# sailab-code/GNN_tf_2.x

Hardware: AMD Instinct MI355X
Metric: node-state-updates/sec (nodes x iters / s), 1M-node synthetic graph (higher is better)
Workload: dtype f32; 1 GPU; synthetic randomGraph-recipe graph, N=1000000 nodes, E=9999690 arcs, state_dim=64, net_state 135->128->128->64 selu+BN, net_output 67->2 softmax+BN, max_iter=30, threshold=0 (all iterations run); the loop-invariant label aggregates (GNN.py:259, :263; 0.2 ms) are kept between Loops until the labels change, see cold_aggregates_ms_per_step; parallelism=single GPU, tile_form=one wave per 32-node tile (k_fused)

## Files before the change

### gnn_tf_2.x_amd/csrc/gnn_fused_kernel.h

```cpp
#pragma once
#include <utility>

#include "gnn_common.h"
#include "gnn_fused.h"

typedef float f32x16 __attribute__((ext_vector_type(16)));

namespace gnn_fused_dev {

#define GNN_GLOBAL __attribute__((address_space(1)))
template <class T>
__device__ __forceinline__ const GNN_GLOBAL T *gptr(const T *p) { return (const GNN_GLOBAL T *)p; }
template <class T>
__device__ __forceinline__ GNN_GLOBAL T *gptr_w(T *p) { return (GNN_GLOBAL T *)p; }
typedef float v4f __attribute__((ext_vector_type(4)));
typedef float v2f __attribute__((ext_vector_type(2)));
typedef int v4i_ __attribute__((ext_vector_type(4)));
__device__ __forceinline__ v4f gload4(const float *p) { return *(const GNN_GLOBAL v4f *)p; }
#ifndef GNN_STORE_AUX
#define GNN_STORE_AUX 2
#endif
__device__ __forceinline__ void gstore_row4(float *base, int64_t off, v4f v)
{
#if GNN_STORE_AUX == 0
// ... 223 lines not shown
#undef GNN_L0_LOAD
#undef GNN_L0_MFMA
}

template <int ACT>
struct ActPipe2 {
    v2f t, u, n, f, p, e;
    static __device__ __forceinline__ v2f splat(float c) { return v2f{c, c}; }
    __device__ __forceinline__ void stage(int st, float v0, float v1, float b0, float b1, float &o0, float &o1)
    {
        if constexpr (ACT == GNN_ACT_SELU) {
            switch (st) {
            case 0: t = v2f{v0, v1} + v2f{b0, b1}; u = t * splat(1.44269504088896341f); break;
            case 1: n = v2f{__builtin_rintf(u.x), __builtin_rintf(u.y)}; f = u - n; break;
            case 2: p = __builtin_elementwise_fma(splat(0.0013218672247603536f), f, splat(0.009671698324382305f));
                    p = __builtin_elementwise_fma(p, f, splat(0.05550893023610115f)); break;
            case 3: p = __builtin_elementwise_fma(p, f, splat(0.24022237956523895f));
                    p = __builtin_elementwise_fma(p, f, splat(0.6931468844413757f)); break;
            case 4: p = __builtin_elementwise_fma(p, f, splat(1.0f)); break;
            case 5: e = v2f{__builtin_ldexpf(p.x, (int)n.x), __builtin_ldexpf(p.y, (int)n.y)}; e = e - splat(1.0f); break;
            case 6: e = e * splat(1.6732632423543772f); break;
            case 7: {
                const v2f r = v2f{t.x > 0.0f ? t.x : e.x, t.y > 0.0f ? t.y : e.y} * splat(1.0507009873554805f);
                o0 = r.x; o1 = r.y;
            } break;
            }
        } else {
            if (st == 0) t = v2f{v0, v1} + v2f{b0, b1};
            if (st == 7) { o0 = gnn_act(t.x, ACT); o1 = gnn_act(t.y, ACT); }
        }
    }
};

template <int NI, int NO, int ACT>
__device__ __forceinline__ void layer_from_regs(f32x16 (&hin)[NI], const float *bias_prev, int half, f32x16 (&acc)[NO],
                                                const float *wp, int wstride)
{
    constexpr int STEPS = 16 * NI, DEPTH = 8;
    float w[STEPS][NO];
#pragma unroll
    for (int s = 0; s < DEPTH; ++s) load_w<NO>(wp + (size_t)s * 64 * NO * wstride, w[s]);
    tile_epilogue<ACT, false>(hin[0], bias_prev, nullptr, nullptr, 0, half);
    acc_to_operand(hin[0]);
    __builtin_amdgcn_sched_barrier(0);
#pragma unroll
    for (int ti = 0; ti < NI; ++ti) {
        float nb[16];
        if (ti + 1 < NI) {
#pragma unroll
            for (int q = 0; q < 4; ++q) {
                const v4f b4 = gload4(bias_prev + 32 * (ti + 1) + 8 * q + 4 * half);
                nb[4 * q] = b4.x; nb[4 * q + 1] = b4.y; nb[4 * q + 2] = b4.z; nb[4 * q + 3] = b4.w;
            }
        }
        __builtin_amdgcn_sched_barrier(0);
        ActPipe2<ACT> ap;
#pragma unroll
        for (int ss = 0; ss < 16; ++ss) {
            const int s = 16 * ti + ss;
            if (s + DEPTH < STEPS) load_w<NO>(wp + (size_t)(s + DEPTH) * 64 * NO * wstride, w[s + DEPTH]);
            const int reg = 4 * (ss >> 2) + ((ss & 3) == 1 ? 2 : (ss & 3) == 2 ? 1 : (ss & 3));
            const float b = hin[ti][reg];
            const bool epi = ti + 1 < NI;
            const int pe = ss & ~1;
#pragma unroll
            for (int jt = 0; jt < NO; ++jt) {
                acc[jt] = __builtin_amdgcn_mfma_f32_32x32x2f32(w[s][jt], b, acc[jt], 0, 0, 0);
                if (epi) {
                    constexpr int SPM = 4 / NO;
#pragma unroll
                    for (int q = jt * SPM; q < (jt + 1) * SPM; ++q) {
                        const int st = (ss & 1) * 4 + q;
                        float o0 = 0.0f, o1 = 0.0f;
                        ap.stage(st, hin[ti + 1][pe], hin[ti + 1][pe + 1], nb[pe], nb[pe + 1], o0, o1);
                        if (st == 7) {
                            auto sw = __builtin_amdgcn_permlane32_swap(__float_as_uint(o0), __float_as_uint(o1), false, false);
                            hin[ti + 1][pe] = __uint_as_float(sw[0]);
                            hin[ti + 1][pe + 1] = __uint_as_float(sw[1]);
                        }
                    }
                }
                __builtin_amdgcn_sched_barrier(0);
            }
            __builtin_amdgcn_sched_barrier(0);
        }
    }
}

typedef int v4i __attribute__((ext_vector_type(4)));
typedef __bf16 bf16x8 __attribute__((ext_vector_type(8)));
__device__ __forceinline__ v4i gload4i(const int *p) { return *(const GNN_GLOBAL v4i *)p; }

__device__ __forceinline__ v4i bload4i(__amdgpu_buffer_rsrc_t r, int voff, int soff)
{
    return __builtin_bit_cast(v4i, __builtin_amdgcn_raw_buffer_load_b128(r, voff, soff, 0));
}
struct WStream {
    int soff, n;
    __device__ __forceinline__ WStream(int start) : soff(start), n(0) {}
    __device__ __forceinline__ v4i next(__amdgpu_buffer_rsrc_t r, int voff)
    {
        if (n == 4) { asm volatile("s_add_u32 %0, %0, 0x1000" : "+s"(soff) : : "scc"); n = 0; }
        return bload4i(r, voff + 1024 * n++, soff);
    }
};

__device__ __forceinline__ f32x16 bias_tile(const float *bias_lds, int jt, int half)
{
    f32x16 t;
#pragma unroll
    for (int q = 0; q < 4; ++q) {
        const v4f b = *reinterpret_cast<const v4f *>(bias_lds + 32 * jt + 8 * q + 4 * half);
        t[4 * q] = b.x; t[4 * q + 1] = b.y; t[4 * q + 2] = b.z; t[4 * q + 3] = b.w;
    }
    return t;
}

__device__ __forceinline__ void split8(const float (&v)[8], v4i &p0, v4i &p1, v4i &p2)
{
#pragma unroll
    for (int j = 0; j < 4; ++j) {
        const unsigned a = __float_as_uint(v[2 * j]), b = __float_as_uint(v[2 * j + 1]);
        const float ar = v[2 * j] - __uint_as_float(a & 0xffff0000u), br = v[2 * j + 1] - __uint_as_float(b & 0xffff0000u);
        const unsigned aru = __float_as_uint(ar), bru = __float_as_uint(br);
        const float ar2 = ar - __uint_as_float(aru & 0xffff0000u), br2 = br - __uint_as_float(bru & 0xffff0000u);
        p0[j] = (int)__builtin_amdgcn_perm(b, a, 0x07060302u);
        p1[j] = (int)__builtin_amdgcn_perm(bru, aru, 0x07060302u);
        p2[j] = (int)__builtin_amdgcn_perm(__float_as_uint(br2), __float_as_uint(ar2), 0x07060302u);
    }
}

__device__ __forceinline__ f32x16 mfma_bf16(v4i a, v4i b, f32x16 c)
{
    return __builtin_amdgcn_mfma_f32_32x32x16_bf16(__builtin_bit_cast(bf16x8, a), __builtin_bit_cast(bf16x8, b), c, 0, 0, 0);
}

__device__ __forceinline__ void split_pair(float v0, float v1, int &p0, int &p1, int &p2)
{
    const unsigned a = __float_as_uint(v0), b = __float_as_uint(v1);
    const float ar = v0 - __uint_as_float(a & 0xffff0000u), br = v1 - __uint_as_float(b & 0xffff0000u);
    const unsigned aru = __float_as_uint(ar), bru = __float_as_uint(br);
    const float ar2 = ar - __uint_as_float(aru & 0xffff0000u), br2 = br - __uint_as_float(bru & 0xffff0000u);
    p0 = (int)__builtin_amdgcn_perm(b, a, 0x07060302u);
    p1 = (int)__builtin_amdgcn_perm(bru, aru, 0x07060302u);
    p2 = (int)__builtin_amdgcn_perm(__float_as_uint(br2), __float_as_uint(ar2), 0x07060302u);
}

typedef _Float16 f16x2 __attribute__((ext_vector_type(2)));
typedef _Float16 f16x8 __attribute__((ext_vector_type(8)));
__device__ __forceinline__ f32x16 mfma_f16(v4i a, v4i b, f32x16 c)
{
    return __builtin_amdgcn_mfma_f32_32x32x16_f16(__builtin_bit_cast(f16x8, a), __builtin_bit_cast(f16x8, b), c, 0, 0, 0);
}
__device__ __forceinline__ void split_pair_f16(float v0, float v1, int &p0, int &p1, float &mx)
{
    constexpr float S = (float)(1 << GNN_F16_EX);
    const v2f s = v2f{v0, v1} * v2f{S, S};
    mx = __builtin_fmaxf(mx, __builtin_fmaxf(__builtin_fabsf(s.x), __builtin_fabsf(s.y)));
    const f16x2 h0 = __builtin_convertvector(s, f16x2);
    const v2f r = s - __builtin_convertvector(h0, v2f);
    const f16x2 h1 = __builtin_convertvector(r, f16x2);
    p0 = __builtin_bit_cast(int, h0);
    p1 = __builtin_bit_cast(int, h1);
}
__device__ __forceinline__ void split8_f16(const float (&v)[8], v4i &p0, v4i &p1, float &mx)
{
#pragma unroll
    for (int j = 0; j < 4; ++j) {
        int q0, q1;
        split_pair_f16(v[2 * j], v[2 * j + 1], q0, q1, mx);
        p0[j] = q0; p1[j] = q1;
    }
}
template <int NI>
__device__ __forceinline__ float hidden_range(const f32x16 (&h)[NI], float us)
{
    float m = 0.0f;
#pragma unroll
    for (int t = 0; t < NI; ++t)
#pragma unroll
        for (int r = 0; r < 16; r += 2) m = __builtin_fmaxf(m, __builtin_fmaxf(__builtin_fabsf(h[t][r]), __builtin_fabsf(h[t][r + 1])));
    return m * (us * (float)(1 << GNN_F16_EX));
}

template <int PC> struct SplitTerms;
template <> struct SplitTerms<3> {
    static constexpr int N = 6;
    static constexpr int PA[6] = {0, 2, 1, 0, 1, 0}, PB[6] = {2, 0, 1, 1, 0, 0};
};
template <> struct SplitTerms<2> {
    static constexpr int N = 3;
    static constexpr int PA[3] = {1, 0, 0}, PB[3] = {0, 1, 0};
};
template <int PC>
__device__ __forceinline__ f32x16 mfma_piece(v4i a, v4i b, f32x16 c)
{
    if constexpr (PC == 2) return mfma_f16(a, b, c);
    else return mfma_bf16(a, b, c);
}
template <int PC>
__device__ __forceinline__ void split8_pc(const float (&v)[8], v4i (&p)[PC], float &mx)
{
    if constexpr (PC == 2) split8_f16(v, p[0], p[1], mx);
    else split8(v, p[0], p[1], p[2]);
}
__device__ __forceinline__ void gnn_flag_raise_range(int *flag_rank_base, float mx)
{
    if (__any(mx >= GNN_F16_LIMIT) && (threadIdx.x & 63) == 0) {
        int *w = flag_rank_base + (blockIdx.x & (GNN_FLAG_SLOTS - 1)) * GNN_FLAG_STRIDE + 3;
        if (__hip_atomic_load(w, __ATOMIC_RELAXED, __HIP_MEMORY_SCOPE_AGENT) == 0) atomicOr(w, 1);
    }
}

template <int T>
__device__ __forceinline__ void mfma_split(const v4i (&w)[T][3], v4i b0, v4i b1, v4i b2, f32x16 *acc)
{
#pragma unroll
    for (int t = 0; t < T; ++t) acc[t] = mfma_bf16(w[t][0], b2, acc[t]);
#pragma unroll
    for (int t = 0; t < T; ++t) acc[t] = mfma_bf16(w[t][2], b0, acc[t]);
#pragma unroll
    for (int t = 0; t < T; ++t) acc[t] = mfma_bf16(w[t][1], b1, acc[t]);
#pragma unroll
    for (int t = 0; t < T; ++t) acc[t] = mfma_bf16(w[t][0], b1, acc[t]);
#pragma unroll
    for (int t = 0; t < T; ++t) acc[t] = mfma_bf16(w[t][1], b0, acc[t]);
#pragma unroll
    for (int t = 0; t < T; ++t) acc[t] = mfma_bf16(w[t][0], b0, acc[t]);
}

template <int NO, bool AL16, int PC = 3>
__device__ __forceinline__ void layer0_split(const float *xr, __amdgpu_buffer_rsrc_t wrs, int voff, int soff, int n_chunks, f32x16 (&acc)[NO],
                                             const float *bias_lds, int half, float &mx)
{
    using TM = SplitTerms<PC>;
    v4i wa[NO][PC], wb[NO][PC];
    float xa[8], xb[8];
    v4i pa[PC], pb[PC];
    WStream ws(soff);
#define GNN_S0_LOAD(W, XV, C)                                                                       \
    _Pragma("unroll") for (int jt = 0; jt < NO; ++jt)                                               \
        _Pragma("unroll") for (int pc = 0; pc < PC; ++pc)                                           \
            W[jt][pc] = ws.next(wrs, voff);                                                         \
    if constexpr (AL16) {                                                                           \
        const v4f lo_ = *reinterpret_cast<const v4f *>(xr + 16 * (C)), hi_ = *reinterpret_cast<const v4f *>(xr + 16 * (C) + 4);   \
        XV[0] = lo_.x; XV[1] = lo_.y; XV[2] = lo_.z; XV[3] = lo_.w; XV[4] = hi_.x; XV[5] = hi_.y; XV[6] = hi_.z; XV[7] = hi_.w;    \
    } else {                                                                                        \
        _Pragma("unroll") for (int i = 0; i < 8; ++i) XV[i] = xr[16 * (C) + i];                     \
    }                                                                                               \
    __builtin_amdgcn_sched_barrier(0);
#define GNN_S0_MFMA(W, P, XN, PN, Z, LIVE)                                                          \
    {                                                                                               \
        float mn_ = 0.0f;                                                                           \
        _Pragma("unroll") for (int term = 0; term < TM::N; ++term)                                  \
            _Pragma("unroll") for (int t = 0; t < NO; ++t) {                                        \
                acc[t] = mfma_piece<PC>(W[t][TM::PA[term]], P[TM::PB[term]], (Z && term == 0) ? bias_tile(bias_lds, t, half) : acc[t]);   \
                const int m = term * NO + t;                                                        \
                constexpr int SL = TM::N * NO - NO;                                                 \
                _Pragma("unroll") for (int j = 0; j < 4; ++j) {                                     \
                    const bool due = PC == 3 ? (m == NO + j) : (m >= NO && (m - NO) == j * SL / 4); \
                    if (due) {                                                                      \
                        if constexpr (PC == 3) {                                                    \
                            int q0, q1, q2;                                                         \
                            split_pair(XN[2 * j], XN[2 * j + 1], q0, q1, q2);                       \
                            PN[0][j] = q0; PN[1][j] = q1; PN[PC - 1][j] = q2;                       \
                        } else {                                                                    \
                            int q0, q1;                                                             \
                            split_pair_f16(XN[2 * j], XN[2 * j + 1], q0, q1, mn_);                  \
                            PN[0][j] = q0; PN[1][j] = q1;                                           \
                        }                                                                           \
                    }                                                                               \
                }                                                                                   \
                __builtin_amdgcn_sched_barrier(0);                                                  \
            }                                                                                       \
        if (PC == 2 && (LIVE)) mx = __builtin_fmaxf(mx, mn_);      \
    }
    GNN_S0_LOAD(wa, xa, 0)
    split8_pc<PC>(xa, pa, mx);
    GNN_S0_LOAD(wb, xb, 1)
    GNN_S0_MFMA(wa, pa, xb, pb, true, 1 < n_chunks)
    for (int c = 1; c < n_chunks; c += 2) {
        GNN_S0_LOAD(wa, xa, c + 1)
        GNN_S0_MFMA(wb, pb, xa, pa, false, c + 1 < n_chunks)
        GNN_S0_LOAD(wb, xb, c + 2)
        if (c + 1 < n_chunks) GNN_S0_MFMA(wa, pa, xb, pb, false, c + 2 < n_chunks)
    }
#undef GNN_S0_LOAD
#undef GNN_S0_MFMA
}

template <int NO, bool AL16>
__device__ __forceinline__ void layer0_split(const float *xr, __amdgpu_buffer_rsrc_t wrs, int voff, int soff, int n_chunks, f32x16 (&acc)[NO],
                                             const float *bias_lds, int half)
{
    float mx = 0.0f;
    layer0_split<NO, AL16, 3>(xr, wrs, voff, soff, n_chunks, acc, bias_lds, half, mx);
}

template <int NI, int NO, int ACT, int PC = 3>
__device__ __forceinline__ void layer_split_from_regs(f32x16 (&hin)[NI], const float *bias_lds, int half, f32x16 (&acc)[NO],
                                                      __amdgpu_buffer_rsrc_t wrs, int voff, int soff, float us, float &mx)
{
    using TM = SplitTerms<PC>;
    constexpr int TPU = NO >= 2 ? 2 : 1, UPC = NO / TPU, CH = 2 * NI, U = CH * UPC;
#ifndef GNN_S1_DEPTH_WIDE
#define GNN_S1_DEPTH_WIDE 1
#endif
    constexpr int DEPTH = (NI + NO >= 8) ? (PC == 2 ? GNN_S1_DEPTH_WIDE : 1) : 3;
    constexpr int NM = TM::N * NO, NTASK = 12;
    v4i w[U][TPU][PC];
    int bp[2][PC][4];
    WStream ws(soff);
#define GNN_S1_LOAD(UU)                                                                             \
    _Pragma("unroll") for (int t = 0; t < TPU; ++t)                                                 \
        _Pragma("unroll") for (int pc = 0; pc < PC; ++pc) w[UU][t][pc] = ws.next(wrs, voff);
#define GNN_S1_H(C, I) hin[(C) >> 1][8 * ((C) & 1) + (I)]
#define GNN_S1_E(C, I)                                                                              \
    if constexpr (ACT == GNN_ACT_SELU) {                                                            \
        constexpr float AL2_ = 1.6732632423543772f * 1.44269504088896341f;                          \
        const float v_ = PC == 2 ? GNN_S1_H(C, I) * us : GNN_S1_H(C, I);                            \
        GNN_S1_H(C, I) = v_ > 0.0f ? v_ : __builtin_fmaf(__builtin_amdgcn_exp2f(v_), AL2_, -AL2_);  \
    } else GNN_S1_H(C, I) = act_fast<ACT>(PC == 2 ? GNN_S1_H(C, I) * us : GNN_S1_H(C, I));
#define GNN_S1_S(C, J, DST)                                                                         \
    if constexpr (PC == 2) { float mz_ = 0.0f; split_pair_f16(GNN_S1_H(C, 2 * (J)), GNN_S1_H(C, 2 * (J) + 1), DST[0][J], DST[1][J], mz_); }   \
    else split_pair(GNN_S1_H(C, 2 * (J)), GNN_S1_H(C, 2 * (J) + 1), DST[0][J], DST[1][J], DST[PC - 1][J]);
#pragma unroll
    for (int u = 0; u < DEPTH && u < U; ++u) { GNN_S1_LOAD(u) }
    {
#pragma unroll
        for (int i = 0; i < 8; ++i) { GNN_S1_E(0, i) }
#pragma unroll
        for (int j = 0; j < 4; ++j) { GNN_S1_S(0, j, bp[0]) }
#pragma unroll
        for (int i = 0; i < 8; ++i) { GNN_S1_E(1, i) }
    }
    __builtin_amdgcn_sched_barrier(0);
#pragma unroll
    for (int c = 0; c < CH; ++c) {
#pragma unroll
        for (int up = 0; up < UPC; ++up) {
            const int u = c * UPC + up;
            if (u + DEPTH < U) { GNN_S1_LOAD(u + DEPTH) }
#pragma unroll
            for (int term = 0; term < TM::N; ++term) {
#pragma unroll
                for (int t = 0; t < TPU; ++t) {
                    const int *bq = bp[c & 1][TM::PB[term]];
                    acc[up * TPU + t] = mfma_piece<PC>(w[u][t][TM::PA[term]], v4i{bq[0], bq[1], bq[2], bq[3]},
                                                  (c == 0 && term == 0) ? bias_tile(bias_lds, up * TPU + t, half) : acc[up * TPU + t]);
                    const int m = (up * TM::N + term) * TPU + t + 1;
                    const int k0 = (m - 1) * NTASK / NM, k1 = m * NTASK / NM;
#pragma unroll
                    for (int k = 0; k < NTASK; ++k) {
                        if (k >= k0 && k < k1) {
                            if (k < 8) { if (c + 2 < CH) { GNN_S1_E(c + 2, k) } }
                            else { if (c + 1 < CH) { GNN_S1_S(c + 1, k - 8, bp[(c + 1) & 1]) } }
                        }
                    }
                    __builtin_amdgcn_sched_barrier(0);
                }
            }
        }
    }
#undef GNN_S1_LOAD
#undef GNN_S1_E
#undef GNN_S1_S
#undef GNN_S1_H
}

template <int NI, int NO, int ACT>
__device__ __forceinline__ void layer_split_from_regs(f32x16 (&hin)[NI], const float *bias_lds, int half, f32x16 (&acc)[NO],
                                                      __amdgpu_buffer_rsrc_t wrs, int voff, int soff)
{
    float mx = 0.0f;
    layer_split_from_regs<NI, NO, ACT, 3>(hin, bias_lds, half, acc, wrs, voff, soff, 1.0f, mx);
}


__device__ __forceinline__ int label_col(int c, int Ds, int NLc, int c_aggs)
{
    return c < NLc ? Ds + c : c_aggs + Ds + (c - NLc);
}

struct RowCol {
    int i, c, qi, qc, width;
    __device__ __forceinline__ RowCol(int lane, int width_) : width(width_)
    {
        i = lane / width; c = lane - i * width;
        qi = 64 / width; qc = 64 - qi * width;
    }
    __device__ __forceinline__ void next()
    {
        i += qi; c += qc;
        if (c >= width) { c -= width; ++i; }
    }
};

__device__ __forceinline__ void zero_pad_columns(const GnnFusedArgs &a, float *X, int lane, int KP)
{
    const int padw = KP - a.in_s;
    RowCol rc(lane, padw);
    for (int t = lane; t < 32 * padw; t += 64, rc.next()) X[rc.i * KP + a.in_s + rc.c] = 0.0f;
    const int hole0 = a.Ds + a.NLc, holew = a.c_aggs - hole0;
    if (holew > 0 && lane < 32)
        for (int c = 0; c < holew; ++c) X[lane * KP + hole0 + c] = 0.0f;
}

template <bool COH = false, int RND = 4>
__device__ __forceinline__ void load_tile_generic(const GnnFusedArgs &a, float *X, const int *ipt, int64_t i0, int lane,
                                               int nvalid, int KP, int c_aggs, bool own_from_lds = false, const int *ecache_src = nullptr,
                                               const float *ecache_w = nullptr, int ecache_base = 0, bool skip_gather = false)
{
    const int Ds = a.Ds, NLc = a.NLc;
    if (!own_from_lds) {
        zero_pad_columns(a, X, lane, KP);
        if (nvalid < 32) {
            RowCol rc(lane, a.in_s);
            for (int t = lane; t < (32 - nvalid) * a.in_s; t += 64, rc.next()) X[(nvalid + rc.i) * KP + rc.c] = 0.0f;
        }
    }
    if (own_from_lds) {
        const int total = nvalid * Ds;
        RowCol rc(lane, Ds);
        for (int t = lane; t < total; t += 64, rc.next()) X[rc.i * KP + rc.c] = X[rc.i * KP + c_aggs + rc.c];
        __builtin_amdgcn_fence(__ATOMIC_ACQ_REL, "wavefront");
    } else {
        const float *src = a.state_cur + (a.row_begin + i0) * Ds;
        const int total = nvalid * Ds;
        RowCol rc(lane, Ds);
        for (int t = lane; t < total; t += 64, rc.next()) X[rc.i * KP + rc.c] = sload1<COH>(src + t);
    }
    if (a.IW > 0 && !own_from_lds) {
        const float *src = a.inv + i0 * a.IW;
        const int total = nvalid * a.IW;
        RowCol rc(lane, a.IW);
        for (int t = lane; t < total; t += 64, rc.next()) X[rc.i * KP + label_col(rc.c, Ds, NLc, c_aggs)] = gload1(src + t);
    }
    __builtin_amdgcn_fence(__ATOMIC_ACQ_REL, "wavefront");
    if (skip_gather) return;
    if (a.agg_in) {
        const float *src = a.agg_in + i0 * Ds;
        const int total = nvalid * Ds;
        RowCol rc(lane, Ds);
        for (int t = lane; t < total; t += 64, rc.next()) X[rc.i * KP + c_aggs + rc.c] = gload1(src + t);
        return;
    }
    if (Ds <= 32) {
        const int node = lane & 31, hf = lane >> 5;
        const int cbeg = hf ? (Ds + 1) / 2 : 0, cend = hf ? Ds : (Ds + 1) / 2;
        const int beg = ipt[node], end = ipt[node + 1];
        float acc[16];
#pragma unroll
        for (int c = 0; c < 16; ++c) acc[c] = 0.0f;
        for (int e = beg; e < end; e += RND) {
            float w[RND];
            const float *xp[RND];
#pragma unroll
            for (int u = 0; u < RND; ++u) {
                const int ee = e + u < end ? e + u : e;
                w[u] = ecache_w ? ecache_w[ee - ecache_base] : gload1(a.adj_w + ee);
                xp[u] = a.state_cur + (int64_t)(ecache_src ? ecache_src[ee - ecache_base] : gload1(a.adj_src + ee)) * Ds + cbeg;
            }
            float x[RND][16];
#pragma unroll
            for (int u = 0; u < RND; ++u)
#pragma unroll
                for (int c = 0; c < 16; ++c) x[u][c] = (cbeg + c < cend) ? sload1<COH>(xp[u] + c) : 0.0f;
#pragma unroll
            for (int u = 0; u < RND; ++u)
                if (e + u < end) {
#pragma unroll
                    for (int c = 0; c < 16; ++c)
                        if (cbeg + c < cend) acc[c] = __builtin_fmaf(w[u], x[u][c], acc[c]);
                }
        }
        if (node < nvalid) {
#pragma unroll
// ... 15 lines not shown
#pragma unroll
            for (int u = 0; u < 4; ++u) {
                const int ee = e + u < end ? e + u : e;
                w[u] = gload1(a.adj_w + ee);
                const float *xp = a.state_cur + (int64_t)gload1(a.adj_src + ee) * Ds + c0;
                if (a.vec == 4) {
                    if constexpr (COH) x[u] = v4f{sload1<true>(xp), sload1<true>(xp + 1), sload1<true>(xp + 2), sload1<true>(xp + 3)};
                    else x[u] = gload4(xp);
                } else x[u] = v4f{sload1<COH>(xp), 0.f, 0.f, 0.f};
            }
#pragma unroll
            for (int u = 0; u < 4; ++u) {
                if (e + u < end) {
                    acc[0] = __builtin_fmaf(w[u], x[u].x, acc[0]);
                    if (a.vec == 4) {
                        acc[1] = __builtin_fmaf(w[u], x[u].y, acc[1]); acc[2] = __builtin_fmaf(w[u], x[u].z, acc[2]);
                        acc[3] = __builtin_fmaf(w[u], x[u].w, acc[3]);
                    }
                }
            }
        }
        if (i < nvalid && colok) {
            float *x = X + i * KP + c_aggs + c0;
            x[0] = acc[0];
            if (a.vec == 4) { x[1] = acc[1]; x[2] = acc[2]; x[3] = acc[3]; }
        }
    }
}

__device__ __forceinline__ void gather_fma(v2f &acc01, v2f &acc23, float w, v4f x)
{
    float a0 = acc01.x, a1 = acc01.y, a2 = acc23.x, a3 = acc23.y;
    asm("v_fma_f32 %0, %1, %2, %0" : "+v"(a0) : "v"(w), "v"(x.x));
    asm("v_fma_f32 %0, %1, %2, %0" : "+v"(a1) : "v"(w), "v"(x.y));
    asm("v_fma_f32 %0, %1, %2, %0" : "+v"(a2) : "v"(w), "v"(x.z));
    asm("v_fma_f32 %0, %1, %2, %0" : "+v"(a3) : "v"(w), "v"(x.w));
    acc01 = v2f{a0, a1}; acc23 = v2f{a2, a3};
}

template <int GB, int... J>
__device__ __forceinline__ void gather_batch(int my_src, float my_w, __amdgpu_buffer_rsrc_t rsrc, int voff0, float (&w)[GB],
                                             v4f (&x)[GB], std::integer_sequence<int, J...>)
{
    ((w[J] = row_bcast_f<J>(my_w),
      x[J] = __builtin_bit_cast(v4f, __builtin_amdgcn_raw_buffer_load_b128(rsrc, (row_bcast_i<J>(my_src) << 8) + voff0, 0, 0))), ...);
}

template <bool AL16>
struct TileOwn64 {
    v4f own[8];
    float lab[4];
    __device__ __forceinline__ void request(const GnnFusedArgs &a, int64_t i0, int lane)
    {
        const float *src = a.state_cur + (a.row_begin + i0) * 64 + lane * 4;
#pragma unroll
        for (int u = 0; u < 8; ++u) own[u] = gload4(src + u * 256);
        const int IW = a.IW, nlab = 32 * IW;
        const float *lsrc = a.inv + i0 * IW;
#pragma unroll
        for (int u = 0; u < 4; ++u) lab[u] = (lane + 64 * u < nlab) ? gload1(lsrc + lane + 64 * u) : 0.0f;
    }
    __device__ __forceinline__ void write(const GnnFusedArgs &a, float *X, int64_t i0, int lane, int KP, int c_aggs) const
    {
        constexpr int Ds = 64;
        const int IW = a.IW, nlab = 32 * IW;
#pragma unroll
        for (int u = 0; u < 8; ++u) {
            float *x = X + (4 * u + (lane >> 4)) * KP + (lane & 15) * 4;
            if constexpr (AL16) *reinterpret_cast<v4f *>(x) = own[u];
            else { x[0] = own[u].x; x[1] = own[u].y; x[2] = own[u].z; x[3] = own[u].w; }
        }
        const float inv_iw = 1.0f / (float)(IW > 0 ? IW : 1);
#pragma unroll
        for (int u = 0; u < 4; ++u) {
            const int t = lane + 64 * u;
            if (t < nlab) {
                const int i = (int)(((float)t + 0.5f) * inv_iw), c = t - i * IW;
                X[i * KP + label_col(c, Ds, a.NLc, c_aggs)] = lab[u];
            }
        }
        if (nlab > 256)
            for (int t = 256 + lane; t < nlab; t += 64) {
                const int i = t / IW, c = t - i * IW;
                X[i * KP + label_col(c, Ds, a.NLc, c_aggs)] = gload1(a.inv + i0 * IW + t);
            }
    }
};

template <bool AL16, bool PADDED = false>
__device__ __forceinline__ void load_tile_fast64(const GnnFusedArgs &a, float *X, const int *ipt, int64_t i0, int lane,
                                                 int KP, int c_aggs, int my_src, float my_w)
{
    constexpr int GB = 16;
    const int gl = lane & 15, grp = lane >> 4;
    TileOwn64<AL16> own;
    own.request(a, i0, lane);
    if constexpr (!PADDED) zero_pad_columns(a, X, lane, KP);
    __builtin_amdgcn_fence(__ATOMIC_ACQ_REL, "wavefront");

    int node = grp * 8;
    const int node_end = node + 8;
    const int e_begin = ipt[node], e_end = ipt[node_end];
    int next_end = ipt[node + 1];
    v2f acc01 = {0.f, 0.f}, acc23 = {0.f, 0.f};
    const __amdgpu_buffer_rsrc_t rsrc = __builtin_amdgcn_make_buffer_rsrc(const_cast<float *>(a.state_cur), 0, (int)a.state_bytes, 0x00020000);
    const int voff0 = gl * 16;
    float *xo = X + c_aggs + gl * 4;
#define GNN_ROW_BOUNDARY(e)                                                                     \
    while ((e) >= next_end) {                                                                   \
        float *xr = xo + node * KP;                                                             \
        if constexpr (AL16) *reinterpret_cast<v4f *>(xr) = v4f{acc01.x, acc01.y, acc23.x, acc23.y};   \
        else { xr[0] = acc01.x; xr[1] = acc01.y; xr[2] = acc23.x; xr[3] = acc23.y; }            \
        acc01 = v2f{0.f, 0.f}; acc23 = v2f{0.f, 0.f};                                           \
        ++node;                                                                                 \
        next_end = ipt[node + 1];                                                               \
    }
    int base = e_begin;
    for (; base + GB <= e_end; base += GB) {
        float w[GB];
        v4f x[GB];
        gather_batch<GB>(my_src, my_w, rsrc, voff0, w, x, std::make_integer_sequence<int, GB>{});
        const int nb = base + GB + gl;
        my_src = 0; my_w = 0.0f;
        if (nb < e_end) { my_src = gstream1(a.adj_src + nb); my_w = gstream1(a.adj_w + nb); }
#pragma unroll
        for (int u = 0; u < GB; ++u) {
            GNN_ROW_BOUNDARY(base + u)
            gather_fma(acc01, acc23, w[u], x[u]);
        }
    }
    {
        const int cnt = e_end - base;
        float w[GB];
        v4f x[GB];
        gather_batch<GB>(my_src, my_w, rsrc, voff0, w, x, std::make_integer_sequence<int, GB>{});
#pragma unroll
        for (int u = 0; u < GB; ++u) {
            if (u < cnt) {
                GNN_ROW_BOUNDARY(base + u)
                gather_fma(acc01, acc23, w[u], x[u]);
            }
        }
    }
#undef GNN_ROW_BOUNDARY
    for (; node < node_end; ++node) {
        float *xr = xo + node * KP;
        if constexpr (AL16) *reinterpret_cast<v4f *>(xr) = v4f{acc01.x, acc01.y, acc23.x, acc23.y};
        else { xr[0] = acc01.x; xr[1] = acc01.y; xr[2] = acc23.x; xr[3] = acc23.y; }
        acc01 = v2f{0.f, 0.f}; acc23 = v2f{0.f, 0.f};
    }
    own.write(a, X, i0, lane, KP, c_aggs);
}

template <bool AL16, int J>
__device__ __forceinline__ void prog_consume(int words, float w, v4f x, v2f &acc01, v2f &acc23, float *xo, int KP)
{
    gather_fma(acc01, acc23, w, x);
    const unsigned t = (unsigned)row_bcast_i<J>(words);
    if (t & GNN_GP_ROW_END) {
        float *xr = xo + __umul24(t & GNN_GP_ROW_MASK, (unsigned)KP);
        if constexpr (AL16) *reinterpret_cast<v4f *>(xr) = v4f{acc01.x, acc01.y, acc23.x, acc23.y};
        else { xr[0] = acc01.x; xr[1] = acc01.y; xr[2] = acc23.x; xr[3] = acc23.y; }
        acc01 = v2f{0.f, 0.f}; acc23 = v2f{0.f, 0.f};
    }
}
template <bool AL16, int GB, int... J>
__device__ __forceinline__ void prog_batch(int words, float my_w, __amdgpu_buffer_rsrc_t rsrc, int voff0, float (&w)[GB], v4f (&x)[GB],
                                           std::integer_sequence<int, J...>)
{
    ((w[J] = row_bcast_f<J>(my_w),
      x[J] = __builtin_bit_cast(v4f, __builtin_amdgcn_raw_buffer_load_b128(rsrc, (row_bcast_i<J>(words) & ~0xff) | voff0, 0, 0))), ...);
}
template <bool AL16, int GB, int... J>
__device__ __forceinline__ void prog_consume_all(int words, const float (&w)[GB], const v4f (&x)[GB], v2f &acc01, v2f &acc23, float *xo, int KP,
                                                 std::integer_sequence<int, J...>)
{
    (prog_consume<AL16, J>(words, w[J], x[J], acc01, acc23, xo, KP), ...);
}
typedef int v2i __attribute__((ext_vector_type(2)));
__device__ __forceinline__ v4i prog_header_request(const GnnFusedArgs &a, int slot)
{
    v4i h = {0, 0, a.gp_slots, 0};
    if (slot < a.gp_slots) h = *reinterpret_cast<const GNN_GLOBAL v4i *>(gptr(a.gp_slot) + 4 * (int64_t)slot);
    return h;
}
__device__ __forceinline__ v2i prog_entry(const GnnFusedArgs &a, int b, int lane)
{
    return *reinterpret_cast<const GNN_GLOBAL v2i *>(gptr(a.gp_ent) + ((int64_t)b * 64 + lane) * 2);
}
template <bool AL16>
__device__ __forceinline__ void load_tile_prog64(const GnnFusedArgs &a, float *X, int64_t i0, int lane, int KP, int c_aggs, int first, int nb, v2i ent)
{
    constexpr int GB = 16;
    const int gl = lane & 15;
    TileOwn64<AL16> own;
    own.request(a, i0, lane);
    v2f acc01 = {0.f, 0.f}, acc23 = {0.f, 0.f};
    const __amdgpu_buffer_rsrc_t rsrc = __builtin_amdgcn_make_buffer_rsrc(const_cast<float *>(a.state_cur), 0, (int)a.state_bytes, 0x00020000);
    const int voff0 = gl * 16;
    float *xo = X + c_aggs + gl * 4;
    for (int b = 0; b < nb; ++b) {
        float w[GB];
        v4f x[GB];
        const int words = ent.x;
        prog_batch<AL16, GB>(words, __int_as_float(ent.y), rsrc, voff0, w, x, std::make_integer_sequence<int, GB>{});
        if (b + 1 < nb) ent = prog_entry(a, first + b + 1, lane);
        prog_consume_all<AL16, GB>(words, w, x, acc01, acc23, xo, KP, std::make_integer_sequence<int, GB>{});
    }
    own.write(a, X, i0, lane, KP, c_aggs);
}

#ifndef GNN_FIRST_BATCH_AHEAD
#define GNN_FIRST_BATCH_AHEAD 1
#endif
template <int GB, int... J>
__device__ __forceinline__ void prog_rows_request(int words, __amdgpu_buffer_rsrc_t rsrc, int voff0, v4f (&x)[GB], std::integer_sequence<int, J...>)
{
    ((x[J] = __builtin_bit_cast(v4f, __builtin_amdgcn_raw_buffer_load_b128(rsrc, (row_bcast_i<J>(words) & ~0xff) | voff0, 0, 0))), ...);
}
template <bool AL16, int GB, int... J>
__device__ __forceinline__ void prog_consume_first(v2i ent, const v4f (&x)[GB], v2f &acc01, v2f &acc23, float *xo, int KP, std::integer_sequence<int, J...>)
{
    (prog_consume<AL16, J>(ent.x, row_bcast_f<J>(__int_as_float(ent.y)), x[J], acc01, acc23, xo, KP), ...);
}
__device__ __forceinline__ void prog_first_batch_request(const GnnFusedArgs &a, int first, int nb, v2i ent0, int lane, v4f (&x0)[16], v2i &ent1)
{
    const __amdgpu_buffer_rsrc_t rsrc = __builtin_amdgcn_make_buffer_rsrc(const_cast<float *>(a.state_cur), 0, (int)a.state_bytes, 0x00020000);
    if (nb > 1) ent1 = prog_entry(a, first + 1, lane);
    __builtin_amdgcn_sched_barrier(0);
    prog_rows_request<16>(ent0.x, rsrc, (lane & 15) * 16, x0, std::make_integer_sequence<int, 16>{});
}
template <bool AL16>
__device__ __forceinline__ void load_tile_prog64_ahead(const GnnFusedArgs &a, float *X, int64_t i0, int lane, int KP, int c_aggs, int first, int nb,
                                                       v2i ent0, const v4f (&x0)[16], v2i ent, v4i hdr_next_raw, int &first_next, int &nb_next,
                                                       int &tid_next, v2i &ent_next)
{
    constexpr int GB = 16;
    const int gl = lane & 15;
    TileOwn64<AL16> own;
    own.request(a, i0, lane);
    v2f acc01 = {0.f, 0.f}, acc23 = {0.f, 0.f};
    const __amdgpu_buffer_rsrc_t rsrc = __builtin_amdgcn_make_buffer_rsrc(const_cast<float *>(a.state_cur), 0, (int)a.state_bytes, 0x00020000);
    const int voff0 = gl * 16;
    float *xo = X + c_aggs + gl * 4;
    auto request_next = [&]() {
        first_next = __builtin_amdgcn_readfirstlane(hdr_next_raw.x); nb_next = __builtin_amdgcn_readfirstlane(hdr_next_raw.y);
        tid_next = __builtin_amdgcn_readfirstlane(hdr_next_raw.z);
        ent = v2i{(int)GNN_GP_NOROW, 0};
        if (nb_next > 0) ent = prog_entry(a, first_next, lane);
    };
    if (nb <= 1) request_next();
    prog_consume_first<AL16, GB>(ent0, x0, acc01, acc23, xo, KP, std::make_integer_sequence<int, GB>{});
    for (int b = 1; b < nb; ++b) {
        float w[GB];
        v4f x[GB];
        const int words = ent.x;
        prog_batch<AL16, GB>(words, __int_as_float(ent.y), rsrc, voff0, w, x, std::make_integer_sequence<int, GB>{});
        if (b + 1 < nb) ent = prog_entry(a, first + b + 1, lane);
        else request_next();
        prog_consume_all<AL16, GB>(words, w, x, acc01, acc23, xo, KP, std::make_integer_sequence<int, GB>{});
    }
    ent_next = ent;
    own.write(a, X, i0, lane, KP, c_aggs);
}

template <bool AL16>
__device__ __forceinline__ void load_tile_given64(const GnnFusedArgs &a, float *X, int64_t i0, int lane, int KP, int c_aggs)
{
    constexpr int Ds = 64;
    v4f own[8], agg[8];
    {
        const float *src = a.state_cur + (a.row_begin + i0) * Ds + lane * 4;
        const float *sag = a.agg_in + i0 * Ds + lane * 4;
#pragma unroll
        for (int u = 0; u < 8; ++u) {
            own[u] = gload4(src + u * 256);
            agg[u] = gload4(sag + u * 256);
        }
    }
    float lab[4];
    const int IW = a.IW, nlab = 32 * IW;
    {
        const float *src = a.inv + i0 * IW;
#pragma unroll
        for (int u = 0; u < 4; ++u) lab[u] = (lane + 64 * u < nlab) ? gload1(src + lane + 64 * u) : 0.0f;
    }
#pragma unroll
    for (int u = 0; u < 8; ++u) {
        float *x = X + (4 * u + (lane >> 4)) * KP + (lane & 15) * 4;
        if constexpr (AL16) { *reinterpret_cast<v4f *>(x) = own[u]; *reinterpret_cast<v4f *>(x + c_aggs) = agg[u]; }
        else {
            x[0] = own[u].x; x[1] = own[u].y; x[2] = own[u].z; x[3] = own[u].w;
            x[c_aggs] = agg[u].x; x[c_aggs + 1] = agg[u].y; x[c_aggs + 2] = agg[u].z; x[c_aggs + 3] = agg[u].w;
        }
    }
    const float inv_iw = 1.0f / (float)(IW > 0 ? IW : 1);
#pragma unroll
    for (int u = 0; u < 4; ++u) {
        const int t = lane + 64 * u;
        if (t < nlab) {
            const int i = (int)(((float)t + 0.5f) * inv_iw), c = t - i * IW;
            X[i * KP + label_col(c, Ds, a.NLc, c_aggs)] = lab[u];
        }
    }
    if (nlab > 256)
        for (int t = 256 + lane; t < nlab; t += 64) {
            const int i = t / IW, c = t - i * IW;
            X[i * KP + label_col(c, Ds, a.NLc, c_aggs)] = gload1(a.inv + i0 * IW + t);
        }
}

template <bool COH = false, bool STORE = true>
__device__ __forceinline__ void check_store_generic(const GnnFusedArgs &a, float *X, int64_t i0, int lane, int nvalid, int KP,
                                                 int c_aggs, int *moved_out = nullptr)
{
    const int Ds = a.Ds, half = lane >> 5;
    if constexpr (STORE) {
        float *dst = a.state_nxt + i0 * Ds;
        const int total = nvalid * Ds;
        RowCol rc(lane, Ds);
        for (int t = lane; t < total; t += 64, rc.next()) sstore1<COH>(dst + t, X[rc.i * KP + c_aggs + rc.c]);
    }
    const float *xo = X + (lane & 31) * KP, *xn = xo + c_aggs;
    float s_ = 0.0f;
    for (int f = 0; f < Ds; ++f) {
        const float o = xo[f];
        const float d = half ? o : (xn[f] - o);
        const float dd = d * d;
        s_ = s_ + dd;
    }
    const float root = sqrtf(s_);
    const float nrm = shfl_f(root, (lane & 31) + 32);
    const float rhs = a.thr * nrm;
    const bool voter = (half == 0) && ((lane & 31) < nvalid);
    const int moved = voter && (root > rhs);
    if (moved_out) *moved_out = __any(moved) ? 1 : 0;
    else if (a.certify) {
        const float band = GNN_BAND_ABS * nrm + GNN_BAND_REL * rhs;
        const int robust = voter && (root > rhs + band), border = voter && gnn_gate_borderline(root, rhs, band);
        const bool am = __any(moved), ar = __any(robust), ab = __any(border);
        if (lane == 0) gnn_flag_raise_certified(a.flag_out, am, ar, ab);
    }
    else if (__any(moved) && lane == 0) gnn_flag_raise(a.flag_out);
}

__device__ __forceinline__ void check_store_fast64(const GnnFusedArgs &a, float *X, int64_t i0, int lane, int KP, int c_aggs)
{
    constexpr int Ds = 64;
    const int half = lane >> 5;
    const float *xo = X + (lane & 31) * KP, *xn = xo + c_aggs;
    float s_ = 0.0f;
#pragma unroll
    for (int f = 0; f < Ds; f += 16) {
        float o[16], nw[16];
#pragma unroll
        for (int u = 0; u < 16; ++u) { o[u] = xo[f + u]; nw[u] = xn[f + u]; }
#pragma unroll
        for (int u = 0; u < 16; ++u) {
            const float d = half ? o[u] : (nw[u] - o[u]);
            const float dd = d * d;
            s_ = s_ + dd;
        }
    }
    const float root = sqrtf(s_);
    const float nrm = shfl_f(root, (lane & 31) + 32);
    const float rhs = a.thr * nrm;
    const int moved = (half == 0) && (root > rhs);
    if (__any(moved) && lane == 0) gnn_flag_raise(a.flag_out);
    float *dst = a.state_nxt + i0 * Ds + lane;
    const float *xs = X + c_aggs + lane;
#pragma unroll
    for (int i = 0; i < 32; i += 8) {
        float v[8];
#pragma unroll
        for (int u = 0; u < 8; ++u) v[u] = xs[(i + u) * KP];
#pragma unroll
// ... 444 lines not shown
```

Before: 1.867 billion node-state-updates/s.

## Micro-optimize f16 split, SELU scaling, range max, and DPP gather FMAs

Several instruction-level tweaks, all on by default. The f16 hi/lo split now computes its residual with v_fma_mix instructions, and hidden_range reduces with v_max3 using abs modifiers. SELU in the f16 path folds the us and f16 scale factors into packed multiplies with an exp2 hoisted ahead of use. The program gather fuses the row broadcast of the weight into v_fmac_f32_dpp row_newbcast and uses leaner address and zeroing code at row ends. These cut VALU instruction count in hot loops, but the inline asm with hand-inserted s_nop hazards may constrain scheduling or give subtly different rounding.

```diff
diff --git a/gnn_tf_2.x_amd/csrc/gnn_fused_kernel.h b/gnn_tf_2.x_amd/csrc/gnn_fused_kernel.h
--- a/gnn_tf_2.x_amd/csrc/gnn_fused_kernel.h
+++ b/gnn_tf_2.x_amd/csrc/gnn_fused_kernel.h
@@ -399,16 +399,31 @@
 {
     return __builtin_amdgcn_mfma_f32_32x32x16_f16(__builtin_bit_cast(f16x8, a), __builtin_bit_cast(f16x8, b), c, 0, 0, 0);
 }
+#ifndef GNN_CUT_FMA_MIX
+#define GNN_CUT_FMA_MIX 1
+#endif
+__device__ __forceinline__ void split_pair_f16_scaled(v2f s, int &p0, int &p1)
+{
+    const f16x2 h0 = __builtin_convertvector(s, f16x2);
+    p0 = __builtin_bit_cast(int, h0);
+#if GNN_CUT_FMA_MIX
+    int q1;
+    asm("v_fma_mixlo_f16 %0, %1, 1.0, -%3 op_sel_hi:[0,0,1]\n\t"
+        "v_fma_mixhi_f16 %0, %2, 1.0, -%3 op_sel:[0,0,1] op_sel_hi:[0,0,1]"
+        : "=&v"(q1) : "v"(s.x), "v"(s.y), "v"(p0));
+    p1 = q1;
+#else
+    const v2f r = s - __builtin_convertvector(h0, v2f);
+    const f16x2 h1 = __builtin_convertvector(r, f16x2);
+    p1 = __builtin_bit_cast(int, h1);
+#endif
+}
 __device__ __forceinline__ void split_pair_f16(float v0, float v1, int &p0, int &p1, float &mx)
 {
     constexpr float S = (float)(1 << GNN_F16_EX);
     const v2f s = v2f{v0, v1} * v2f{S, S};
     mx = __builtin_fmaxf(mx, __builtin_fmaxf(__builtin_fabsf(s.x), __builtin_fabsf(s.y)));
-    const f16x2 h0 = __builtin_convertvector(s, f16x2);
-    const v2f r = s - __builtin_convertvector(h0, v2f);
-    const f16x2 h1 = __builtin_convertvector(r, f16x2);
-    p0 = __builtin_bit_cast(int, h0);
-    p1 = __builtin_bit_cast(int, h1);
+    split_pair_f16_scaled(s, p0, p1);
 }
 __device__ __forceinline__ void split8_f16(const float (&v)[8], v4i &p0, v4i &p1, float &mx)
 {
@@ -419,6 +434,9 @@
         p0[j] = q0; p1[j] = q1;
     }
 }
+#ifndef GNN_RANGE_MAX3
+#define GNN_RANGE_MAX3 1
+#endif
 template <int NI>
 __device__ __forceinline__ float hidden_range(const f32x16 (&h)[NI], float us)
 {
@@ -426,7 +444,14 @@
 #pragma unroll
     for (int t = 0; t < NI; ++t)
 #pragma unroll
-        for (int r = 0; r < 16; r += 2) m = __builtin_fmaxf(m, __builtin_fmaxf(__builtin_fabsf(h[t][r]), __builtin_fabsf(h[t][r + 1])));
+        for (int r = 0; r < 16; r += 2) {
+#if GNN_RANGE_MAX3
+            if (t == 0 && r == 0) asm("s_nop 7\n\ts_nop 7\n\ts_nop 3\n\tv_max3_f32 %0, |%1|, |%2|, %0" : "+v"(m) : "v"(h[t][r]), "v"(h[t][r + 1]));
+            else asm("v_max3_f32 %0, |%1|, |%2|, %0" : "+v"(m) : "v"(h[t][r]), "v"(h[t][r + 1]));
+#else
+            m = __builtin_fmaxf(m, __builtin_fmaxf(__builtin_fabsf(h[t][r]), __builtin_fabsf(h[t][r + 1])));
+#endif
+        }
     return m * (us * (float)(1 << GNN_F16_EX));
 }
 
@@ -562,14 +587,35 @@
     _Pragma("unroll") for (int t = 0; t < TPU; ++t)                                                 \
         _Pragma("unroll") for (int pc = 0; pc < PC; ++pc) w[UU][t][pc] = ws.next(wrs, voff);
 #define GNN_S1_H(C, I) hin[(C) >> 1][8 * ((C) & 1) + (I)]
+#ifndef GNN_SELU_ONE_SCALE
+#define GNN_SELU_ONE_SCALE 1
+#endif
+    constexpr bool PRESCALED = GNN_SELU_ONE_SCALE && PC == 2 && ACT == GNN_ACT_SELU;
+    [[maybe_unused]] float ex_[CH][8];
+    [[maybe_unused]] v2f usv_ = {us, us}, us16v_ = {us * (float)(1 << GNN_F16_EX), us * (float)(1 << GNN_F16_EX)};
+    if constexpr (PRESCALED) asm("" : "+v"(usv_), "+v"(us16v_));
 #define GNN_S1_E(C, I)                                                                              \
-    if constexpr (ACT == GNN_ACT_SELU) {                                                            \
+    if constexpr (PRESCALED) {                                                                      \
+        constexpr float AL16_ = 1.6732632423543772f * 1.44269504088896341f * (float)(1 << GNN_F16_EX);   \
+        if (((I) & 1) == 0) {                                                                       \
+            const v2f h_ = v2f{GNN_S1_H(C, (I) & ~1), GNN_S1_H(C, (I) | 1)};                        \
+            const v2f m_ = h_ * usv_, s_ = h_ * us16v_;                                             \
+            ex_[C][(I) & ~1] = __builtin_amdgcn_exp2f(m_.x); ex_[C][(I) | 1] = __builtin_amdgcn_exp2f(m_.y);   \
+            GNN_S1_H(C, (I) & ~1) = s_.x; GNN_S1_H(C, (I) | 1) = s_.y;                              \
+        } else {                                                                                    \
+            _Pragma("unroll") for (int i_ = (I) - 1; i_ <= (I); ++i_) {                             \
+                const float s_ = GNN_S1_H(C, i_);                                                   \
+                GNN_S1_H(C, i_) = s_ > 0.0f ? s_ : __builtin_fmaf(ex_[C][i_], AL16_, -AL16_);       \
+            }                                                                                       \
+        }                                                                                           \
+    } else if constexpr (ACT == GNN_ACT_SELU) {                                                     \
         constexpr float AL2_ = 1.6732632423543772f * 1.44269504088896341f;                          \
         const float v_ = PC == 2 ? GNN_S1_H(C, I) * us : GNN_S1_H(C, I);                            \
         GNN_S1_H(C, I) = v_ > 0.0f ? v_ : __builtin_fmaf(__builtin_amdgcn_exp2f(v_), AL2_, -AL2_);  \
     } else GNN_S1_H(C, I) = act_fast<ACT>(PC == 2 ? GNN_S1_H(C, I) * us : GNN_S1_H(C, I));
 #define GNN_S1_S(C, J, DST)                                                                         \
-    if constexpr (PC == 2) { float mz_ = 0.0f; split_pair_f16(GNN_S1_H(C, 2 * (J)), GNN_S1_H(C, 2 * (J) + 1), DST[0][J], DST[1][J], mz_); }   \
+    if constexpr (PRESCALED) split_pair_f16_scaled(v2f{GNN_S1_H(C, 2 * (J)), GNN_S1_H(C, 2 * (J) + 1)}, DST[0][J], DST[1][J]);   \
+    else if constexpr (PC == 2) { float mz_ = 0.0f; split_pair_f16(GNN_S1_H(C, 2 * (J)), GNN_S1_H(C, 2 * (J) + 1), DST[0][J], DST[1][J], mz_); }   \
     else split_pair(GNN_S1_H(C, 2 * (J)), GNN_S1_H(C, 2 * (J) + 1), DST[0][J], DST[1][J], DST[PC - 1][J]);
 #pragma unroll
     for (int u = 0; u < DEPTH && u < U; ++u) { GNN_S1_LOAD(u) }
@@ -891,23 +937,59 @@
     own.write(a, X, i0, lane, KP, c_aggs);
 }
 
+#ifndef GNN_GATHER_FMAC_DPP
+#define GNN_GATHER_FMAC_DPP 1
+#endif
+#ifndef GNN_ROW_END_LEAN
+#define GNN_ROW_END_LEAN 1
+#endif
+template <int J>
+__device__ __forceinline__ void gather_fmac_bcast(v2f &acc01, v2f &acc23, float my_w, v4f x)
+{
+    float a0 = acc01.x, a1 = acc01.y, a2 = acc23.x, a3 = acc23.y;
+#define GNN_FMAC_DPP_(D, X) "v_fmac_f32_dpp " D ", %4, " X " row_newbcast:%9 row_mask:0xf bank_mask:0xf bound_ctrl:1\n\t"
+    if constexpr (J == 0)
+        asm("s_nop 1\n\t" GNN_FMAC_DPP_("%0", "%5") GNN_FMAC_DPP_("%1", "%6") GNN_FMAC_DPP_("%2", "%7") GNN_FMAC_DPP_("%3", "%8")
+            : "+v"(a0), "+v"(a1), "+v"(a2), "+v"(a3) : "v"(my_w), "v"(x.x), "v"(x.y), "v"(x.z), "v"(x.w), "n"(J));
+    else
+        asm(GNN_FMAC_DPP_("%0", "%5") GNN_FMAC_DPP_("%1", "%6") GNN_FMAC_DPP_("%2", "%7") GNN_FMAC_DPP_("%3", "%8")
+            : "+v"(a0), "+v"(a1), "+v"(a2), "+v"(a3) : "v"(my_w), "v"(x.x), "v"(x.y), "v"(x.z), "v"(x.w), "n"(J));
+#undef GNN_FMAC_DPP_
+    acc01 = v2f{a0, a1}; acc23 = v2f{a2, a3};
+}
 template <bool AL16, int J>
 __device__ __forceinline__ void prog_consume(int words, float w, v4f x, v2f &acc01, v2f &acc23, float *xo, int KP)
 {
+#if GNN_GATHER_FMAC_DPP
+    gather_fmac_bcast<J>(acc01, acc23, w, x);
+#else
     gather_fma(acc01, acc23, w, x);
+#endif
     const unsigned t = (unsigned)row_bcast_i<J>(words);
     if (t & GNN_GP_ROW_END) {
+#if GNN_ROW_END_LEAN
+        float *xr = reinterpret_cast<float *>(reinterpret_cast<char *>(xo) + __umul24(t & GNN_GP_ROW_MASK, 4u * (unsigned)KP));
+#else
         float *xr = xo + __umul24(t & GNN_GP_ROW_MASK, (unsigned)KP);
+#endif
         if constexpr (AL16) *reinterpret_cast<v4f *>(xr) = v4f{acc01.x, acc01.y, acc23.x, acc23.y};
         else { xr[0] = acc01.x; xr[1] = acc01.y; xr[2] = acc23.x; xr[3] = acc23.y; }
+#if GNN_ROW_END_LEAN
+        asm("v_mov_b64 %0, 0\n\tv_mov_b64 %1, 0" : "=v"(acc01), "=v"(acc23));
+#else
         acc01 = v2f{0.f, 0.f}; acc23 = v2f{0.f, 0.f};
+#endif
     }
 }
 template <bool AL16, int GB, int... J>
 __device__ __forceinline__ void prog_batch(int words, float my_w, __amdgpu_buffer_rsrc_t rsrc, int voff0, float (&w)[GB], v4f (&x)[GB],
                                            std::integer_sequence<int, J...>)
 {
+#if GNN_GATHER_FMAC_DPP
+    ((w[J] = my_w,
+#else
     ((w[J] = row_bcast_f<J>(my_w),
+#endif
       x[J] = __builtin_bit_cast(v4f, __builtin_amdgcn_raw_buffer_load_b128(rsrc, (row_bcast_i<J>(words) & ~0xff) | voff0, 0, 0))), ...);
 }
 template <bool AL16, int GB, int... J>
@@ -960,7 +1042,11 @@
 template <bool AL16, int GB, int... J>
 __device__ __forceinline__ void prog_consume_first(v2i ent, const v4f (&x)[GB], v2f &acc01, v2f &acc23, float *xo, int KP, std::integer_sequence<int, J...>)
 {
+#if GNN_GATHER_FMAC_DPP
+    (prog_consume<AL16, J>(ent.x, __int_as_float(ent.y), x[J], acc01, acc23, xo, KP), ...);
+#else
     (prog_consume<AL16, J>(ent.x, row_bcast_f<J>(__int_as_float(ent.y)), x[J], acc01, acc23, xo, KP), ...);
+#endif
 }
 __device__ __forceinline__ void prog_first_batch_request(const GnnFusedArgs &a, int first, int nb, v2i ent0, int lane, v4f (&x0)[16], v2i &ent1)
 {
```

Result: no change. 1.882 billion node-state-updates/s (median of 6 runs) (+0.8%).
